# KTH-RPL/cloth-splatting

Measured on AMD Instinct MI355X. Metric: rasterizer fwd+bwd rendered Mpix/s (scene_1, 800x800), higher is better.
Workload: dtype f32

## Files before the change

cloth-splatting_amd/csrc/csplat_image.hip:

```cpp
#include "csplat_common.h"
#include <math.h>
#include <stdlib.h>

namespace {
constexpr int BW = 64, BH = 16, R5 = 5;
struct Taps { float w[11]; };

__global__ __launch_bounds__(256) void k_blur11(int H, int W, Taps taps, const float *__restrict__ in, float *__restrict__ out) {
    __shared__ float s_in[(BH + 2 * R5)][BW + 2 * R5 + 1];
    __shared__ float s_h[(BH + 2 * R5)][BW + 1];
    const size_t img = (size_t)blockIdx.z * H * W;
    const int x0 = blockIdx.x * BW, y0 = blockIdx.y * BH;
    for (int t = threadIdx.x; t < (BH + 2 * R5) * (BW + 2 * R5); t += 256) {
        const int ry = t / (BW + 2 * R5), rx = t - ry * (BW + 2 * R5);
        const int y = y0 + ry - R5, x = x0 + rx - R5;
        s_in[ry][rx] = (y >= 0 && y < H && x >= 0 && x < W) ? in[img + (size_t)y * W + x] : 0.f;
    }
    __syncthreads();
    for (int t = threadIdx.x; t < (BH + 2 * R5) * BW; t += 256) {
        const int ry = t / BW, rx = t - ry * BW;
        float a = 0.f;
#pragma unroll
        for (int k = 0; k < 11; k++) a += taps.w[k] * s_in[ry][rx + k];
        s_h[ry][rx] = a;
// ... 326 lines not shown
#pragma unroll
        for (int o = 32; o > 0; o >>= 1) t += __shfl_xor(t, o, 64);
        __syncthreads();
        if ((threadIdx.x & 63) == 0) s_red[threadIdx.x >> 6] = t;
        __syncthreads();
        float r = 0.f;
        for (int k = 0; k < SSIM_THREADS / 64; k++) r += s_red[k];
        return r;
    };
    const float ssim_sum = block_sum(partial, 0, nwg);
    const float l1_sum = block_sum(partial + nwg, 0, nwg);
    const int n_batch = planes / channels;
    double psnr_sum = 0.0;
    for (int b = 0; b < n_batch; b++) {
        const float q = block_sum(partial + 2 * nwg, (size_t)b * channels * per_plane, (size_t)(b + 1) * channels * per_plane);
        const float mse = q / ((float)channels * (float)H * (float)W);
        psnr_sum += (double)(20.f * log10f(1.f / sqrtf(mse)));
    }
    if (threadIdx.x == 0) {
        const float n = (float)planes * (float)H * (float)W;
        const float l1 = l1_sum / n;
        const float image_loss = masked ? l1 + lam * (ssim_sum / n) : l1 + lam * (1.f - ssim_sum / n);
        out[0] = img_weight * image_loss + (add ? add_weight * add[0] : 0.f);
        out[1] = psnr_scale * (float)psnr_sum;
        out[2] = image_loss;
        out[3] = l1;
    }
}

constexpr int L1_BLOCKS = 256, L1_THREADS = 1024;
__global__ __launch_bounds__(L1_THREADS) void k_l1(int64_t n, const float *__restrict__ a, const float *__restrict__ b,
                                                    float inv_n, float *__restrict__ partial, float *__restrict__ grad,
                                                    const float *__restrict__ mask, int64_t hw, int channels, int mask_channels,
                                                    signed char *__restrict__ sign8) {
    __shared__ float s_red[L1_THREADS / 64];
    float acc = 0.f;
    auto sg = [&](float d) { return d > 0.f ? inv_n : (d < 0.f ? -inv_n : 0.f); };
    auto s8 = [&](float d) { return (signed char)(d > 0.f ? 1 : (d < 0.f ? -1 : 0)); };
    auto moff = [&](int64_t e) {
        const int64_t plane = e / hw;
        return (mask_channels == 1 ? plane / channels : plane) * hw + (e - plane * hw);
    };
    const bool al = ((((uintptr_t)a | (uintptr_t)b | (uintptr_t)grad | (uintptr_t)mask) & 15u) == 0);
    const int64_t n4 = ((mask && (hw & 3)) || !al) ? 0 : n >> 2;
    auto one = [&](int64_t i, const float4 x, const float4 y) {
        float d0 = x.x - y.x, d1 = x.y - y.y, d2 = x.z - y.z, d3 = x.w - y.w;
        if (mask) {
            const float4 m = *reinterpret_cast<const float4 *>(mask + moff(i << 2));
            d0 *= m.x; d1 *= m.y; d2 *= m.z; d3 *= m.w;
            acc += (fabsf(d0) + fabsf(d1)) + (fabsf(d2) + fabsf(d3));
            if (grad) reinterpret_cast<float4 *>(grad)[i] = make_float4(sg(d0) * m.x, sg(d1) * m.y, sg(d2) * m.z, sg(d3) * m.w);
        } else {
            acc += (fabsf(d0) + fabsf(d1)) + (fabsf(d2) + fabsf(d3));
            if (grad) reinterpret_cast<float4 *>(grad)[i] = make_float4(sg(d0), sg(d1), sg(d2), sg(d3));
        }
        if (sign8) reinterpret_cast<char4 *>(sign8)[i] = make_char4(s8(d0), s8(d1), s8(d2), s8(d3));
    };
    const int64_t stride = (int64_t)gridDim.x * L1_THREADS;
    int64_t i = (int64_t)blockIdx.x * L1_THREADS + threadIdx.x;
    for (; i + 3 * stride < n4; i += 4 * stride) {
        const float4 x0 = reinterpret_cast<const float4 *>(a)[i], y0 = reinterpret_cast<const float4 *>(b)[i];
        const float4 x1 = reinterpret_cast<const float4 *>(a)[i + stride], y1 = reinterpret_cast<const float4 *>(b)[i + stride];
        const float4 x2 = reinterpret_cast<const float4 *>(a)[i + 2 * stride], y2 = reinterpret_cast<const float4 *>(b)[i + 2 * stride];
        const float4 x3 = reinterpret_cast<const float4 *>(a)[i + 3 * stride], y3 = reinterpret_cast<const float4 *>(b)[i + 3 * stride];
        one(i, x0, y0);
        one(i + stride, x1, y1);
        one(i + 2 * stride, x2, y2);
        one(i + 3 * stride, x3, y3);
    }
    for (; i + stride < n4; i += 2 * stride) {
        const float4 x0 = reinterpret_cast<const float4 *>(a)[i], y0 = reinterpret_cast<const float4 *>(b)[i];
        const float4 x1 = reinterpret_cast<const float4 *>(a)[i + stride], y1 = reinterpret_cast<const float4 *>(b)[i + stride];
        one(i, x0, y0);
        one(i + stride, x1, y1);
    }
    if (i < n4) one(i, reinterpret_cast<const float4 *>(a)[i], reinterpret_cast<const float4 *>(b)[i]);
    for (int64_t i = (n4 << 2) + (int64_t)blockIdx.x * L1_THREADS + threadIdx.x; i < n; i += (int64_t)gridDim.x * L1_THREADS) {
        float d = a[i] - b[i];
        float m = 1.f;
        if (mask) { m = mask[moff(i)]; d *= m; }
        acc += fabsf(d);
        if (grad) grad[i] = sg(d) * m;
        if (sign8) sign8[i] = s8(d);
    }
#pragma unroll
    for (int o = 32; o > 0; o >>= 1) acc += __shfl_xor(acc, o, 64);
    if ((threadIdx.x & 63) == 0) s_red[threadIdx.x >> 6] = acc;
    __syncthreads();
    if (threadIdx.x == 0) { float t_ = 0.f; for (int k_ = 0; k_ < L1_THREADS / 64; k_++) t_ += s_red[k_]; partial[blockIdx.x] = t_; }
}
__global__ __launch_bounds__(L1_BLOCKS) void k_l1_finish(int nparts, const float *__restrict__ partial, float inv_n, float *__restrict__ loss) {
    __shared__ float s[L1_BLOCKS];
    s[threadIdx.x] = (int)threadIdx.x < nparts ? partial[threadIdx.x] : 0.f;
    __syncthreads();
    if (threadIdx.x == 0) {
        float tt = 0.f;
        for (int g = 0; g < L1_BLOCKS / 16; g++) {
            float t = 0.f;
            for (int k = 0; k < 16; k++) t += s[16 * g + k];
            tt += t;
        }
        *loss = tt * inv_n;
    }
}
constexpr int GL_THREADS = 256, GL_MAX_BLOCKS = 1024, GL_VIEWS = 16;
struct GeomTable {
    const float *D[GL_VIEWS], *A[GL_VIEWS], *Z[GL_VIEWS], *S[GL_VIEWS], *M[GL_VIEWS];
};
__device__ __forceinline__ unsigned geom_code(float r, float w) {
    if (r != r || w != w) return 3u;
    const int sr = (r > 0.f) - (r < 0.f), sw = (w > 0.f) - (w < 0.f);
    return (unsigned)(sr * sw + 1);
}
__device__ __forceinline__ float geom_sign(unsigned code) { return code == 3u ? __builtin_nanf("") : (float)((int)code - 1); }
__device__ __forceinline__ bool geom_valid(float z) { return z > 0.f && z < __builtin_inff(); }

template <bool HAS_Z, bool HAS_S>
__device__ __forceinline__ unsigned geom_pixel(float d, float a, float z, float s, float m, float &acc_d, float &acc_s) {
    unsigned code_d = 1u, code_s = 1u;
    if (HAS_Z) {
        const float w = geom_valid(z) ? m : 0.f;
        const bool on = w != 0.f;
        const float r = fmaf(-a, z, d);
        acc_d += on ? fabsf(r * w) : 0.f;
        code_d = on ? geom_code(r, w) : 1u;
    }
    if (HAS_S) {
        const bool on = m != 0.f;
        const float r = a - s;
        acc_s += on ? fabsf(r * m) : 0.f;
        code_s = on ? geom_code(r, m) : 1u;
    }
    return code_d | (code_s << 2);
}

// ... 167 lines not shown
__global__ __launch_bounds__(256) void k_l1_bwd(int64_t n, const signed char *__restrict__ sign8, const float *__restrict__ g, float inv_n,
                                                const float *__restrict__ mask, int64_t hw, int channels, int mask_channels,
                                                float *__restrict__ out) {
    const float sc = g[0] * inv_n;
    auto moff = [&](int64_t e) {
        const int64_t plane = e / hw;
        return (mask_channels == 1 ? plane / channels : plane) * hw + (e - plane * hw);
    };
    const int64_t n4 = ((mask && (hw & 3)) || ((uintptr_t)mask & 15u)) ? 0 : n >> 2;
    const int64_t stride = (int64_t)gridDim.x * 256;
    for (int64_t i = (int64_t)blockIdx.x * 256 + threadIdx.x; i < n4; i += stride) {
        const char4 s = reinterpret_cast<const char4 *>(sign8)[i];
        float4 o = make_float4(sc * (float)s.x, sc * (float)s.y, sc * (float)s.z, sc * (float)s.w);
        if (mask) {
            const float4 m = *reinterpret_cast<const float4 *>(mask + moff(i << 2));
            o.x *= m.x; o.y *= m.y; o.z *= m.z; o.w *= m.w;
        }
        reinterpret_cast<float4 *>(out)[i] = o;
    }
    for (int64_t i = (n4 << 2) + (int64_t)blockIdx.x * 256 + threadIdx.x; i < n; i += stride)
        out[i] = sc * (float)sign8[i] * (mask ? mask[moff(i)] : 1.f);
}

static int l1_launch(void *stream, int64_t n, const float *a, const float *b, void *scratch, float *loss, float *grad,
                     const float *mask, int64_t hw, int channels, int mask_channels, const char *who, signed char *sign8 = nullptr) {
    CSPLAT_REQUIRE(n > 0 && a && b && scratch && loss, "csplat_l1: bad arguments");
    CSPLAT_REQUIRE((((uintptr_t)a | (uintptr_t)b | (uintptr_t)grad | (uintptr_t)mask) & 3u) == 0, "csplat_l1: operands must be 4-byte aligned");
    const bool al = ((((uintptr_t)a | (uintptr_t)b | (uintptr_t)grad | (uintptr_t)mask) & 15u) == 0);
    float *partial = (float *)scratch;
    const int64_t units = ((mask && (hw & 3)) || !al) ? n : n / 4;
    const int64_t work = (units + L1_THREADS - 1) / L1_THREADS;
    const int grid = (int)(work < 1 ? 1 : (work > L1_BLOCKS ? L1_BLOCKS : work));
    CSPLAT_REQUIRE(((uintptr_t)sign8 & 3u) == 0, "csplat_l1: the sign buffer must be 4-byte aligned");
    k_l1<<<grid, L1_THREADS, 0, (hipStream_t)stream>>>(n, a, b, 1.0f / (float)n, partial, grad, mask, hw, channels, mask_channels, sign8);
    LAUNCH_CHECK();
    k_l1_finish<<<1, L1_BLOCKS, 0, (hipStream_t)stream>>>(grid, partial, 1.0f / (float)n, loss);
    LAUNCH_CHECK();
    (void)who;
    return 0;
}

extern "C" int csplat_l1(void *stream, int64_t n, const float *a, const float *b, void *scratch, float *loss, float *grad) {
    return l1_launch(stream, n, a, b, scratch, loss, grad, nullptr, 1, 1, 1, "csplat_l1");
}

extern "C" int csplat_l1_masked(void *stream, int64_t n_batch, int channels, int64_t hw, const float *a, const float *b,
                                const float *mask, int mask_channels, void *scratch, float *loss, float *grad) {
    CSPLAT_REQUIRE(n_batch > 0 && channels > 0 && hw > 0 && mask, "csplat_l1_masked: bad arguments");
    CSPLAT_REQUIRE(mask_channels == 1 || mask_channels == channels, "csplat_l1_masked: the mask has 1 plane per image or one per channel");
    return l1_launch(stream, n_batch * channels * hw, a, b, scratch, loss, grad, mask, hw, channels, mask_channels, "csplat_l1_masked");
}

extern "C" int csplat_l1_signs(void *stream, int64_t n_batch, int channels, int64_t hw, const float *a, const float *b, const float *mask,
                               int mask_channels, void *scratch, float *loss, signed char *sign8) {
    CSPLAT_REQUIRE(n_batch > 0 && channels > 0 && hw > 0 && sign8, "csplat_l1_signs: bad arguments");
    CSPLAT_REQUIRE(!mask || mask_channels == 1 || mask_channels == channels, "csplat_l1_signs: the mask has 1 plane per image or one per channel");
    return l1_launch(stream, n_batch * channels * hw, a, b, scratch, loss, nullptr, mask, hw, channels, mask ? mask_channels : 1, "csplat_l1_signs", sign8);
}
extern "C" int csplat_l1_signs_bwd(void *stream, int64_t n_batch, int channels, int64_t hw, const signed char *sign8, const float *mask,
                                   int mask_channels, const float *g_scalar, float *out) {
    CSPLAT_REQUIRE(n_batch > 0 && channels > 0 && hw > 0 && sign8 && g_scalar && out, "csplat_l1_signs_bwd: bad arguments");
    CSPLAT_REQUIRE(((uintptr_t)out & 15u) == 0 && (((uintptr_t)sign8 | (uintptr_t)mask) & 3u) == 0, "csplat_l1_signs_bwd: operands must be aligned");
    const int64_t n = n_batch * channels * hw;
    const int64_t work = (n / 4 + 255) / 256;
    const int grid = (int)(work < 1 ? 1 : (work > 4096 ? 4096 : work));
    k_l1_bwd<<<grid, 256, 0, (hipStream_t)stream>>>(n, sign8, g_scalar, 1.0f / (float)n, mask, hw, channels, mask ? mask_channels : 1, out);
    LAUNCH_CHECK();
    return 0;
}
// ... 209 lines not shown
```

cloth-splatting_amd/csrc/csplat_raster.hip:

```cpp
#include "csplat_common.h"

#include <atomic>
#include <cstring>
#include <chrono>
#include <mutex>
#include <type_traits>

#include "csplat_raster_math.h"
#include "csplat_raster_k1.h"
#include "csplat_raster_binning.h"
#include "csplat_raster_k5b_k6.h"

namespace {

constexpr int ACC_STRIDE = 16;

#define CSPLAT_ROWMASK_OP(OP, dst, src0, src1, RM)                                                                                  \
    asm("s_nop 1\n\tv_" OP "_f32_dpp %0, %1, %2 quad_perm:[0,1,2,3] row_mask:" RM " bank_mask:0xf" : "+v"(dst) : "v"(src0), "v"(src1))
__device__ __forceinline__ void rows_scan_mul(float f, float Tin, float &Tr, float &Tout) {
    const auto s16 = __builtin_amdgcn_permlane16_swap(__float_as_uint(f), __float_as_uint(f), false, false);
    const float ev = __uint_as_float(s16[0]), od = __uint_as_float(s16[1]);
    const float pr = ev * od;
    const auto s32 = __builtin_amdgcn_permlane32_swap(__float_as_uint(pr), __float_as_uint(pr), false, false);
    const float lo = __uint_as_float(s32[0]), hi = __uint_as_float(s32[1]);
// ... 730 lines not shown
        std::lock_guard<std::mutex> lk(g_ticket_mu);
        for (int i = 0; i < MAX_TICKETS && tk < 0; i++)
            if (!g_tickets[i].used) tk = i;
        if (tk >= 0) g_tickets[tk].used = true;
    }
    CSPLAT_REQUIRE(tk >= 0, "csplat_forward_begin: more than 64 forwards begun and not finished");
    FwdTicket &t = g_tickets[tk];
    t.s = s; t.P = P; t.W = W; t.H = H; t.tiles = tiles; t.nb = cdiv(P > 0 ? P : 1, BUCKET_G); t.can_bucket = can_bucket;
    t.use_mail = false; t.tag = 0; t.mb_host = nullptr; t.mb_dev = nullptr;
    if (can_bucket && !dbg(CSPLAT_DEBUG_NO_MAILBOX) && mail_init()) {
        t.use_mail = true;
        t.tag = g_mail.next.fetch_add(1);
        if (t.tag == 0) t.tag = g_mail.next.fetch_add(1);
        const int slot = (int)(t.tag % MAIL_SLOTS);
        t.mb_host = g_mail.host + slot * MAIL_WORDS;
        t.mb_dev = g_mail.dev + slot * MAIL_WORDS;
    }
    t.cam = cam; t.g = geom_view(gbase, P); t.gbase = gbase; t.ibase = ibase;
    t.ranges = im.ranges; t.n_contrib = im.n_contrib; t.final_T = im.final_T; t.info = im.info;
    t.table = table; t.bg = bg; t.radii = radii; t.alloc = alloc; t.alloc_ctx = alloc_ctx;
    t.D = D; t.M = M; t.means3D = means3D; t.shs = shs; t.colors_precomp = colors_precomp; t.opacities = opacities; t.scales = scales;
    t.scale_modifier = scale_modifier; t.rotations = rotations; t.cov3D_precomp = cov3D_precomp;
    t.aa = (prefiltered & CSPLAT_ANTIALIAS) != 0;
    *ticket_out = tk;
    return 0;
}

static int nocull_mode() { return dbg(CSPLAT_DEBUG_NO_CULLING) ? 1 : dbg(CSPLAT_DEBUG_CULL_RADIUS_X4) ? 2 : 0; }

static int begin_launch(const FwdTicket &t) {
    hipStream_t s = t.s;
    const int P = t.P, tiles = t.tiles, nb = t.nb;
    if (!t.can_bucket) HIP_TRY(hipMemsetAsync(t.ranges, 0, (size_t)tiles * 8, s));
    if (P > 0) {
        ProfScope ps(PROF_K1, s);
        const bool stage = t.shs != nullptr && t.M == 16 && ((uintptr_t)t.shs & 15u) == 0;
        if (t.aa && stage)
            k_preprocess_aa<true><<<cdiv(P, 256), 256, 0, s>>>(P, t.D, t.M, t.means3D, t.shs, t.colors_precomp, t.opacities, t.scales,
                                                                t.scale_modifier, t.rotations, t.cov3D_precomp, t.cam, t.g, t.radii, nocull_mode());
        else if (t.aa)
            k_preprocess_aa<false><<<cdiv(P, 256), 256, 0, s>>>(P, t.D, t.M, t.means3D, t.shs, t.colors_precomp, t.opacities, t.scales,
                                                                 t.scale_modifier, t.rotations, t.cov3D_precomp, t.cam, t.g, t.radii, nocull_mode());
        else if (stage)
            k_preprocess<true><<<cdiv(P, 256), 256, 0, s>>>(P, t.D, t.M, t.means3D, t.shs, t.colors_precomp, t.opacities, t.scales,
                                                             t.scale_modifier, t.rotations, t.cov3D_precomp, t.cam, t.g, t.radii, nocull_mode());
        else
            k_preprocess<false><<<cdiv(P, 256), 256, 0, s>>>(P, t.D, t.M, t.means3D, t.shs, t.colors_precomp, t.opacities, t.scales,
                                                              t.scale_modifier, t.rotations, t.cov3D_precomp, t.cam, t.g, t.radii, nocull_mode());
        LAUNCH_CHECK();
    }
    if (t.can_bucket) {
        ProfScope ps(PROF_K2, s);
        if (P > 0) {
            k_tile_count<<<nb, BUCKET_G, (size_t)tiles * 4, s>>>(P, tiles, t.g.xy, t.radii, t.cam, t.table);
            LAUNCH_CHECK();
        } else {
            HIP_TRY(hipMemsetAsync(t.table, 0, (size_t)nb * tiles * 4, s));
        }
        uint32_t *tile_cnt = t.table + (size_t)nb * tiles;
        k_tile_colscan<<<cdiv(tiles, 256), 256, 0, s>>>(tiles, nb, t.table, tile_cnt);
        LAUNCH_CHECK();
        k_tile_scan<<<1, 1024, 0, s>>>(tiles, tile_cnt, t.ranges, t.info, t.mb_dev, t.tag);
        LAUNCH_CHECK();
    }
    return 0;
}

static bool begin_views_compatible(int V, const int *tk) {
    if (V < 1 || V > RASTER_MAX_VIEWS || dbg(CSPLAT_DEBUG_PER_VIEW_LAUNCHES)) return false;
    const FwdTicket &a = g_tickets[tk[0]];
    if (a.P <= 0 || !a.can_bucket || !a.shs || a.colors_precomp || a.cov3D_precomp || !a.scales || !a.rotations) return false;
    for (int i = 1; i < V; i++) {
        const FwdTicket &w = g_tickets[tk[i]];
        if (w.P != a.P || w.D != a.D || w.M != a.M || w.W != a.W || w.H != a.H || w.shs != a.shs || w.opacities != a.opacities ||
            w.scales != a.scales || w.scale_modifier != a.scale_modifier || w.colors_precomp || w.cov3D_precomp || !w.rotations ||
            !w.can_bucket || w.aa != a.aa)
            return false;
    }
    return true;
}
static int begin_launch_views(int V, const int *tk, hipStream_t join) {
    const FwdTicket &a = g_tickets[tk[0]];
    const int P = a.P, tiles = a.tiles, nb = a.nb;
    K1Table tab;
    tab.n = V;
    for (int i = 0; i < V; i++) {
        const FwdTicket &t = g_tickets[tk[i]];
        K1View &k = tab.v[i];
        k.means3D = t.means3D; k.rotations = t.rotations; k.cam = t.cam; k.g = t.g; k.radii = t.radii; k.table = t.table;
        k.info = t.info; k.mailbox = t.mb_dev; k.ranges = t.ranges; k.tag = t.tag;
    }
    {
        ProfScope ps(PROF_K1, join);
        const bool stage = a.M == 16 && ((uintptr_t)a.shs & 15u) == 0;
        if (a.aa && stage)
            k_preprocess_views_aa<true><<<cdiv(P, K1V_G), 256, 0, join>>>(P, a.D, a.M, a.shs, a.opacities, a.scales, a.scale_modifier, tab,
                                                                        nocull_mode());
        else if (a.aa)
            k_preprocess_views_aa<false><<<cdiv(P, K1V_G), 256, 0, join>>>(P, a.D, a.M, a.shs, a.opacities, a.scales, a.scale_modifier, tab,
                                                                         nocull_mode());
        else if (stage)
            k_preprocess_views<true><<<cdiv(P, K1V_G), 256, 0, join>>>(P, a.D, a.M, a.shs, a.opacities, a.scales, a.scale_modifier, tab,
                                                                     nocull_mode());
        else
            k_preprocess_views<false><<<cdiv(P, K1V_G), 256, 0, join>>>(P, a.D, a.M, a.shs, a.opacities, a.scales, a.scale_modifier, tab,
                                                                      nocull_mode());
        LAUNCH_CHECK();
    }
    {
        ProfScope ps(PROF_K2, join);
        k_tile_count_views<<<dim3(nb, V), BUCKET_G, (size_t)tiles * 4, join>>>(P, tiles, tab);
        LAUNCH_CHECK();
        k_tile_colscan_views<<<dim3(cdiv(tiles, 256), V), 256, 0, join>>>(tiles, nb, tab);
        LAUNCH_CHECK();
        k_tile_scan_views<<<V, 1024, 0, join>>>(tiles, nb, tab);
        LAUNCH_CHECK();
    }
    return 0;
}

int csplat_forward_begin(void *stream, int P, int D, int M, const float *bg, int W, int H, const float *means3D,
                         const float *shs, const float *colors_precomp, const float *opacities, const float *scales,
                         float scale_modifier, const float *rotations, const float *cov3D_precomp, const float *view,
                         const float *proj, const float *campos, float tanfovx, float tanfovy, int prefiltered,
                         csplat_alloc_fn alloc, void *alloc_ctx, int32_t *radii, int *ticket_out) {
    CSPLAT_REQUIRE(!(prefiltered & CSPLAT_ANTIALIAS), "csplat_forward / csplat_forward_begin: CSPLAT_ANTIALIAS needs a csplat_view entry point "
                                                      "(csplat_forward_views*), whose backward knows the bit");
    if (int rc = begin_prepare(stream, P, D, M, bg, W, H, means3D, shs, colors_precomp, opacities, scales, scale_modifier, rotations,
                               cov3D_precomp, view, proj, campos, tanfovx, tanfovy, prefiltered, alloc, alloc_ctx, radii, ticket_out))
        return rc;
    const int rc = begin_launch(g_tickets[*ticket_out]);
    if (rc) {
        std::lock_guard<std::mutex> lk(g_ticket_mu);
        g_tickets[*ticket_out].used = false;
    }
    return rc;
}

static int finish_read(const FwdTicket &t, uint32_t host_info[3], hipStream_t launched_on = nullptr) {
    hipStream_t s = launched_on ? launched_on : t.s;
    host_info[0] = host_info[1] = host_info[2] = 0;
    if (t.can_bucket) {
        bool got = false;
        if (t.use_mail) {
            const auto t0 = std::chrono::steady_clock::now();
            unsigned spins = 0;
            while (!(got = (t.mb_host[2] == t.tag))) {
                if ((++spins & 0x3FFu) == 0 &&
// ... 1134 lines not shown
```

cloth-splatting_amd/csrc/csplat_raster_binning.h:

```cpp
#pragma once

namespace {

__global__ __launch_bounds__(256) void k_emit_keys(int P, const float2 *__restrict__ xy, const float *__restrict__ depth,
                                                    const uint32_t *__restrict__ offsets,
                                                    const int32_t *__restrict__ radii, Cam cam,
                                                    uint64_t *__restrict__ keys, uint32_t *__restrict__ ids) {
    const int i = blockIdx.x * blockDim.x + threadIdx.x;
    if (i >= P) return;
    const int rad = radii[i];
    if (rad <= 0) return;
    uint32_t off = (i == 0) ? 0u : offsets[i - 1];
    const float2 p = xy[i];
    int minx, miny, maxx, maxy;
    tile_rect(p.x, p.y, rad, cam, minx, miny, maxx, maxy);
    const uint32_t dbits = __float_as_uint(depth[i]);
    for (int y = miny; y < maxy; y++)
        for (int x = minx; x < maxx; x++) {
            keys[off] = ((uint64_t)(uint32_t)(y * cam.gx + x) << 32) | dbits;
            ids[off] = (uint32_t)i;
            off++;
        }
}

__global__ __launch_bounds__(256) void k_tile_ranges(int64_t R, const uint64_t *__restrict__ keys, int2 *__restrict__ ranges) {
    const int64_t i = (int64_t)blockIdx.x * blockDim.x + threadIdx.x;
    if (i >= R) return;
    const uint32_t t = (uint32_t)(keys[i] >> 32);
    if (i == 0) ranges[t].x = 0;
    else {
        const uint32_t tp = (uint32_t)(keys[i - 1] >> 32);
        if (tp != t) { ranges[tp].y = (int)i; ranges[t].x = (int)i; }
    }
    if (i == R - 1) ranges[t].y = (int)R;
}

constexpr int BUCKET_CAP = 8192;
constexpr int BUCKET_TILES = 12288;
constexpr int BUCKET_G = 1024;

__device__ __forceinline__ void tile_count_body(int P, int tiles, const float2 *__restrict__ xy,
                                                const int32_t *__restrict__ radii, const Cam &cam,
                                                uint32_t *__restrict__ table) {
    extern __shared__ uint32_t s_hist[];
    for (int t = threadIdx.x; t < tiles; t += BUCKET_G) s_hist[t] = 0u;
    __syncthreads();
    const int i = blockIdx.x * BUCKET_G + threadIdx.x;
    if (i < P) {
        const int rad = radii[i];
        if (rad > 0) {
            const float2 p = xy[i];
            int minx, miny, maxx, maxy;
            tile_rect(p.x, p.y, rad, cam, minx, miny, maxx, maxy);
            for (int y = miny; y < maxy; y++)
                for (int x = minx; x < maxx; x++) atomicAdd(&s_hist[y * cam.gx + x], 1u);
        }
    }
    __syncthreads();
    uint32_t *row = table + (size_t)blockIdx.x * tiles;
    for (int t = threadIdx.x; t < tiles; t += BUCKET_G) row[t] = s_hist[t];
}
__global__ __launch_bounds__(BUCKET_G) void k_tile_count(int P, int tiles, const float2 *__restrict__ xy,
                                                          const int32_t *__restrict__ radii, Cam cam,
                                                          uint32_t *__restrict__ table) {
    tile_count_body(P, tiles, xy, radii, cam, table);
}
__global__ __launch_bounds__(BUCKET_G) void k_tile_count_views(int P, int tiles, K1Table tab) {
    const K1View &w = tab.v[blockIdx.y];
    tile_count_body(P, tiles, w.g.xy, w.radii, w.cam, w.table);
}

__device__ __forceinline__ void tile_colscan_body(int tiles, int nb, uint32_t *__restrict__ table, uint32_t *__restrict__ cnt) {
    const int t = blockIdx.x * 256 + threadIdx.x;
    if (t >= tiles) return;
    uint32_t run = 0;
    int b = 0;
    for (; b + 8 <= nb; b += 8) {
        uint32_t v[8];
#pragma unroll
        for (int u = 0; u < 8; u++) v[u] = table[(size_t)(b + u) * tiles + t];
#pragma unroll
        for (int u = 0; u < 8; u++) { table[(size_t)(b + u) * tiles + t] = run; run += v[u]; }
    }
    for (; b < nb; b++) { const uint32_t v = table[(size_t)b * tiles + t]; table[(size_t)b * tiles + t] = run; run += v; }
    cnt[t] = run;
}
__global__ __launch_bounds__(256) void k_tile_colscan(int tiles, int nb, uint32_t *__restrict__ table, uint32_t *__restrict__ cnt) {
    tile_colscan_body(tiles, nb, table, cnt);
}
__global__ __launch_bounds__(256) void k_tile_colscan_views(int tiles, int nb, K1Table tab) {
    uint32_t *table = tab.v[blockIdx.y].table;
    tile_colscan_body(tiles, nb, table, table + (size_t)nb * tiles);
}

constexpr int INFO_BUSY = 64;
constexpr int LPT_BINS = 512;
constexpr int TSCAN_ITEMS = BUCKET_TILES / 1024;
__device__ __forceinline__ void tile_scan_body(int tiles, const uint32_t *__restrict__ cnt, int2 *__restrict__ ranges,
                                               uint32_t *__restrict__ info, volatile uint32_t *mailbox, uint32_t tag) {
    __shared__ unsigned long long s_w[17];
    __shared__ uint32_t s_max[16];
    __shared__ uint32_t s_bin[LPT_BINS + 1];
    const int lane = threadIdx.x & 63, w = threadIdx.x >> 6;
    uint32_t *busy = info + INFO_BUSY;
    uint32_t *lpt = busy + tiles + 4;
    const int per = (tiles + 1023) / 1024, t0 = threadIdx.x * per;
    uint32_t c[TSCAN_ITEMS];
#pragma unroll
    for (int k = 0; k < TSCAN_ITEMS; k++) c[k] = (k < per && t0 + k < tiles) ? cnt[t0 + k] : 0u;
    for (int i = threadIdx.x; i <= LPT_BINS; i += 1024) s_bin[i] = 0u;
    uint32_t mx = 0;
    unsigned long long v0 = 0ull;
#pragma unroll
    for (int k = 0; k < TSCAN_ITEMS; k++) { mx = max(mx, c[k]); v0 += (unsigned long long)c[k] | ((unsigned long long)(c[k] ? 1u : 0u) << 32); }
    unsigned long long inc = v0;
#pragma unroll
    for (int d = 1; d < 64; d <<= 1) { const unsigned long long o = __shfl_up(inc, d, 64); if (lane >= d) inc += o; }
    if (lane == 63) s_w[w] = inc;
    __syncthreads();
    if (w == 0) {
        unsigned long long v = lane < 16 ? s_w[lane] : 0ull, vi = v;
#pragma unroll
        for (int d = 1; d < 16; d <<= 1) { const unsigned long long o = __shfl_up(vi, d, 64); if (lane >= d) vi += o; }
        if (lane < 16) s_w[lane] = vi - v;
        if (lane == 15) s_w[16] = vi;
    }
    __syncthreads();
    const unsigned long long carry = s_w[16];
    {
        unsigned long long exl = s_w[w] + inc - v0;
#pragma unroll
        for (int k = 0; k < TSCAN_ITEMS; k++) {
            const int t = t0 + k;
            if (k < per && t < tiles) {
                const uint32_t ex = (uint32_t)exl, nz = (uint32_t)(exl >> 32);
                ranges[t] = c[k] ? make_int2((int)ex, (int)(ex + c[k])) : make_int2(0, 0);
                if (c[k]) {
                    busy[1 + nz] = (uint32_t)t;
                    atomicAdd(&s_bin[LPT_BINS - 1 - min(c[k] >> 4, (uint32_t)(LPT_BINS - 1))], 1u);
                } else {
                    lpt[tiles - 1 - (t - (int)nz)] = (uint32_t)t;
                }
// ... 9 lines not shown
            for (int k = 0; k < LPT_BINS / 64; k++) { v[k] = s_bin[lane * (LPT_BINS / 64) + k]; run += v[k]; }
            uint32_t binc = run;
#pragma unroll
            for (int d = 1; d < 64; d <<= 1) { const uint32_t o = (uint32_t)__shfl_up((int)binc, d, 64); if (lane >= d) binc += o; }
            uint32_t base = binc - run;
#pragma unroll
            for (int k = 0; k < LPT_BINS / 64; k++) { s_bin[lane * (LPT_BINS / 64) + k] = base; base += v[k]; }
        }
        __syncthreads();
#pragma unroll
        for (int k = 0; k < TSCAN_ITEMS; k++)
            if (c[k]) lpt[atomicAdd(&s_bin[LPT_BINS - 1 - min(c[k] >> 4, (uint32_t)(LPT_BINS - 1))], 1u)] = (uint32_t)(t0 + k);
    }
#pragma unroll
    for (int d = 32; d > 0; d >>= 1) mx = max(mx, (uint32_t)__shfl_xor((int)mx, d, 64));
    if (lane == 0) s_max[w] = mx;
    __syncthreads();
    if (threadIdx.x == 0) {
        uint32_t m = 0;
        for (int k = 0; k < 16; k++) m = max(m, s_max[k]);
        info[0] = (uint32_t)carry;
        info[1] = m;
        info[2] = (uint32_t)(carry >> 32);
        busy[0] = (uint32_t)(carry >> 32);
        if (mailbox) {
            mailbox[0] = (uint32_t)carry;
            mailbox[1] = m;
            mailbox[3] = (uint32_t)(carry >> 32);
            __threadfence_system();
            mailbox[2] = tag;
        }
    }
}
__global__ __launch_bounds__(1024) void k_tile_scan(int tiles, const uint32_t *__restrict__ cnt, int2 *__restrict__ ranges,
                                                     uint32_t *__restrict__ info, volatile uint32_t *mailbox, uint32_t tag) {
    tile_scan_body(tiles, cnt, ranges, info, mailbox, tag);
}
__global__ __launch_bounds__(1024) void k_tile_scan_views(int tiles, int nb, K1Table tab) {
    const K1View &w = tab.v[blockIdx.x];
    tile_scan_body(tiles, w.table + (size_t)nb * tiles, w.ranges, w.info, w.mailbox, w.tag);
}

__device__ __forceinline__ void emit_bucket_body(int P, int tiles, const float2 *__restrict__ xy,
                                                 const float *__restrict__ depth, const int32_t *__restrict__ radii,
                                                 const Cam &cam, const uint32_t *__restrict__ table,
                                                 const int2 *__restrict__ ranges, uint64_t *__restrict__ comp) {
    extern __shared__ uint32_t s_base[];
    const uint32_t *row = table + (size_t)blockIdx.x * tiles;
    for (int t = threadIdx.x; t < tiles; t += BUCKET_G) s_base[t] = (uint32_t)ranges[t].x + row[t];
    __syncthreads();
    const int i = blockIdx.x * BUCKET_G + threadIdx.x;
    if (i >= P) return;
    const int rad = radii[i];
    if (rad <= 0) return;
    const float2 p = xy[i];
    int minx, miny, maxx, maxy;
    tile_rect(p.x, p.y, rad, cam, minx, miny, maxx, maxy);
    const uint64_t v = ((uint64_t)__float_as_uint(depth[i]) << 32) | (uint32_t)i;
    for (int y = miny; y < maxy; y++)
        for (int x = minx; x < maxx; x++) comp[atomicAdd(&s_base[y * cam.gx + x], 1u)] = v;
}
__global__ __launch_bounds__(BUCKET_G) void k_emit_bucket(int P, int tiles, const float2 *__restrict__ xy,
                                                           const float *__restrict__ depth, const int32_t *__restrict__ radii,
                                                           Cam cam, const uint32_t *__restrict__ table,
                                                           const int2 *__restrict__ ranges, uint64_t *__restrict__ comp) {
    emit_bucket_body(P, tiles, xy, depth, radii, cam, table, ranges, comp);
}

struct P2View {
    Geom g;
    Cam cam;
    const int32_t *radii;
    const uint32_t *table;
// ... 393 lines not shown
```

cloth-splatting_amd/csrc/csplat_raster_k1.h:

```cpp
#pragma once

namespace {

template <bool STAGE, bool AA = false>
__device__ __forceinline__ void preprocess_body(int P, int D, int M, const float *__restrict__ means3D,
                                                const float *__restrict__ shs,
                                                const float *__restrict__ colors_precomp,
                                                const float *__restrict__ opacities,
                                                const float *__restrict__ scales, float scale_mod,
                                                const float *__restrict__ rotations,
                                                const float *__restrict__ cov3D_precomp, const Cam &cam, const Geom &g,
                                                int32_t *__restrict__ radii, int nocull, const float *s_shrows, int i, int srow) {
#pragma clang fp contract(off)
    if (i >= P) return;
    float depth = 0.f, px = 0.f, py = 0.f, cut = -1.f;
    float4 co = {0.f, 0.f, 0.f, 0.f};
    float rgb[3] = {0.f, 0.f, 0.f};
    float c6[6] = {0.f, 0.f, 0.f, 0.f, 0.f, 0.f};
    uint32_t clampbits = 0, touched = 0;
    int rad = 0;

    const float p[3] = {means3D[3 * i], means3D[3 * i + 1], means3D[3 * i + 2]};
    float pv[3];
    view_point(p, cam.view, pv);
// ... 71 lines not shown
                if (res < 0.f) clampbits |= (1u << ch);
                rgb[ch] = fmaxf(res, 0.f);
            }
        }
        depth = pv[2];
        rad = r;
        px = ix; py = iy;
        float op = opacities[i];
        if constexpr (AA) op = op * aa_h;
        co = make_float4(c * det_inv, -b * det_inv, a * det_inv, op);
        touched = (uint32_t)((maxy - miny) * (maxx - minx));
        const float cancel = 4e-7f * (a * c + b * b) / det;
        cut = cancel < 0.25f ? 2.f * lam1 * logf(255.f * op) * (1.0001f + 2.f * cancel) + 0.01f : 3.0e38f;
        if (nocull == 1) cut = 3.0e38f;
        if (nocull == 2) cut = cut * 4.f + 4.f;
    } while (0);

    g.depth[i] = depth;
    radii[i] = rad;
    g.xy[i] = make_float2(px, py);
    g.conic_opacity[i] = co;
#pragma unroll
    for (int k = 0; k < 3; k++) g.rgb[3 * i + k] = rgb[k];
#pragma unroll
    for (int k = 0; k < 6; k++) g.cov3D[6 * i + k] = c6[k];
    g.clamped[i] = clampbits;
    g.tiles_touched[i] = touched;
    g.cut2[i] = cut;
    g.pack[3 * (size_t)i] = make_float4(px, py, co.x, co.y);
    g.pack[3 * (size_t)i + 1] = make_float4(co.z, co.w, rgb[0], rgb[1]);
    g.pack[3 * (size_t)i + 2] = make_float4(rgb[2], depth, cut, 0.f);
}

template <bool STAGE>
__global__ __launch_bounds__(256) void k_preprocess(int P, int D, int M, const float *__restrict__ means3D,
                                                     const float *__restrict__ shs,
                                                     const float *__restrict__ colors_precomp,
                                                     const float *__restrict__ opacities,
                                                     const float *__restrict__ scales, float scale_mod,
                                                     const float *__restrict__ rotations,
                                                     const float *__restrict__ cov3D_precomp, Cam cam, Geom g,
                                                     int32_t *__restrict__ radii, int nocull) {
    __shared__ float s_shrows[STAGE ? 256 * SH_ROW : 1];
    if (STAGE) {
        const int base = blockIdx.x * 256;
        stage_sh_rows<256>(shs + (size_t)base * 48, min(256, P - base), s_shrows);
        __syncthreads();
    }
    preprocess_body<STAGE>(P, D, M, means3D, shs, colors_precomp, opacities, scales, scale_mod, rotations, cov3D_precomp, cam, g, radii,
                           nocull, s_shrows, (int)(blockIdx.x * blockDim.x + threadIdx.x), (int)threadIdx.x);
}
template <bool STAGE>
__global__ __launch_bounds__(256) void k_preprocess_aa(int P, int D, int M, const float *__restrict__ means3D,
                                                        const float *__restrict__ shs,
                                                        const float *__restrict__ colors_precomp,
                                                        const float *__restrict__ opacities,
                                                        const float *__restrict__ scales, float scale_mod,
                                                        const float *__restrict__ rotations,
                                                        const float *__restrict__ cov3D_precomp, Cam cam, Geom g,
                                                        int32_t *__restrict__ radii, int nocull) {
    __shared__ float s_shrows[STAGE ? 256 * SH_ROW : 1];
    if (STAGE) {
        const int base = blockIdx.x * 256;
        stage_sh_rows<256>(shs + (size_t)base * 48, min(256, P - base), s_shrows);
        __syncthreads();
    }
    preprocess_body<STAGE, true>(P, D, M, means3D, shs, colors_precomp, opacities, scales, scale_mod, rotations, cov3D_precomp, cam, g,
                                 radii, nocull, s_shrows, (int)(blockIdx.x * blockDim.x + threadIdx.x), (int)threadIdx.x);
}

struct K1View {
    const float *means3D, *rotations;
    Cam cam;
    Geom g;
    int32_t *radii;
    uint32_t *table, *info, *mailbox;
    int2 *ranges;
    uint32_t tag;
};
struct K1Table { int n; K1View v[RASTER_MAX_VIEWS]; };

constexpr int K1V_G = 64;
template <bool STAGE>
__global__ __launch_bounds__(256) void k_preprocess_views(int P, int D, int M, const float *__restrict__ shs,
                                                           const float *__restrict__ opacities,
                                                           const float *__restrict__ scales, float scale_mod, K1Table tab,
                                                           int nocull) {
    __shared__ float s_shrows[STAGE ? K1V_G * SH_ROW : 1];
    const int base = blockIdx.x * K1V_G;
    if (STAGE) {
        stage_sh_rows<256>(shs + (size_t)base * 48, min(K1V_G, P - base), s_shrows);
        __syncthreads();
    }
    const int lane = threadIdx.x & 63;
    for (int vi = threadIdx.x >> 6; vi < tab.n; vi += 4) {
        const K1View &w = tab.v[vi];
        preprocess_body<STAGE>(P, D, M, w.means3D, shs, nullptr, opacities, scales, scale_mod, w.rotations, nullptr, w.cam, w.g, w.radii, nocull,
                               s_shrows, base + lane, lane);
    }
}
template <bool STAGE>
__global__ __launch_bounds__(256) void k_preprocess_views_aa(int P, int D, int M, const float *__restrict__ shs,
                                                              const float *__restrict__ opacities,
                                                              const float *__restrict__ scales, float scale_mod, K1Table tab,
                                                              int nocull) {
    __shared__ float s_shrows[STAGE ? K1V_G * SH_ROW : 1];
    const int base = blockIdx.x * K1V_G;
    if (STAGE) {
        stage_sh_rows<256>(shs + (size_t)base * 48, min(K1V_G, P - base), s_shrows);
        __syncthreads();
    }
    const int lane = threadIdx.x & 63;
    for (int vi = threadIdx.x >> 6; vi < tab.n; vi += 4) {
        const K1View &w = tab.v[vi];
        preprocess_body<STAGE, true>(P, D, M, w.means3D, shs, nullptr, opacities, scales, scale_mod, w.rotations, nullptr, w.cam, w.g, w.radii,
                                     nocull, s_shrows, base + lane, lane);
    }
}

}
```

Before: 4737.

## Fuse tile histogram, column scan and tile scan via atomics and last-block ticket

Replaces the three-kernel binning sequence (per-block tile histogram, column-wise exclusive scan, single-block tile scan) with one kernel. Each block atomically adds its per-tile counts into a global total and keeps the returned base as its offset, and the last block to draw a ticket runs the tile scan. Tile totals and the ticket are zeroed inside the preprocess kernel. The L1 loss finish kernel is likewise folded into the main reduction using a last-block ticket. Both remove kernel launches and the separate colscan pass over memory. In exchange, per-block offsets become nondeterministic, so primitive order within a tile now depends on atomic ordering, and correctness relies on cross-block memory-ordering assumptions.

Result: no change. 4700 (-0.8%).

```diff
diff --git a/cloth-splatting_amd/csrc/csplat_image.hip b/cloth-splatting_amd/csrc/csplat_image.hip
--- a/cloth-splatting_amd/csrc/csplat_image.hip
+++ b/cloth-splatting_amd/csrc/csplat_image.hip
@@ -382,7 +382,7 @@
 __global__ __launch_bounds__(L1_THREADS) void k_l1(int64_t n, const float *__restrict__ a, const float *__restrict__ b,
                                                     float inv_n, float *__restrict__ partial, float *__restrict__ grad,
                                                     const float *__restrict__ mask, int64_t hw, int channels, int mask_channels,
-                                                    signed char *__restrict__ sign8) {
+                                                    signed char *__restrict__ sign8, float *__restrict__ loss) {
     __shared__ float s_red[L1_THREADS / 64];
     float acc = 0.f;
     auto sg = [&](float d) { return d > 0.f ? inv_n : (d < 0.f ? -inv_n : 0.f); };
@@ -437,20 +437,35 @@
     for (int o = 32; o > 0; o >>= 1) acc += __shfl_xor(acc, o, 64);
     if ((threadIdx.x & 63) == 0) s_red[threadIdx.x >> 6] = acc;
     __syncthreads();
-    if (threadIdx.x == 0) { float t_ = 0.f; for (int k_ = 0; k_ < L1_THREADS / 64; k_++) t_ += s_red[k_]; partial[blockIdx.x] = t_; }
-}
-__global__ __launch_bounds__(L1_BLOCKS) void k_l1_finish(int nparts, const float *__restrict__ partial, float inv_n, float *__restrict__ loss) {
-    __shared__ float s[L1_BLOCKS];
-    s[threadIdx.x] = (int)threadIdx.x < nparts ? partial[threadIdx.x] : 0.f;
-    __syncthreads();
+    uint32_t *ticket = reinterpret_cast<uint32_t *>(partial + L1_BLOCKS);
     if (threadIdx.x == 0) {
-        float tt = 0.f;
-        for (int g = 0; g < L1_BLOCKS / 16; g++) {
-            float t = 0.f;
-            for (int k = 0; k < 16; k++) t += s[16 * g + k];
-            tt += t;
-        }
+        float t_ = 0.f;
+        for (int k_ = 0; k_ < L1_THREADS / 64; k_++) t_ += s_red[k_];
+        __hip_atomic_store(partial + blockIdx.x, t_, __ATOMIC_RELAXED, __HIP_MEMORY_SCOPE_AGENT);
+    }
+    if (threadIdx.x < 64) asm volatile("s_waitcnt vmcnt(0)" ::: "memory");
+    __syncthreads();
+    if (threadIdx.x >= 64) return;
+    uint32_t drawn = 0u;
+    if (threadIdx.x == 0) drawn = __hip_atomic_fetch_add(ticket, 1u, __ATOMIC_RELAXED, __HIP_MEMORY_SCOPE_AGENT);
+    if ((uint32_t)__builtin_amdgcn_readfirstlane((int)drawn) != gridDim.x - 1) return;
+    float t = 0.f;
+    if (threadIdx.x < L1_BLOCKS / 16) {
+        float v[16];
+#pragma unroll
+        for (int k = 0; k < 16; k++) {
+            const unsigned idx = 16u * threadIdx.x + k;
+            v[k] = __hip_atomic_load(partial + idx, __ATOMIC_RELAXED, __HIP_MEMORY_SCOPE_AGENT);
+        }
+#pragma unroll
+        for (int k = 0; k < 16; k++) t += 16u * threadIdx.x + k < gridDim.x ? v[k] : 0.f;
+    }
+    float tt = 0.f;
+#pragma unroll
+    for (int g = 0; g < L1_BLOCKS / 16; g++) tt += __shfl(t, g, 64);
+    if (threadIdx.x == 0) {
         *loss = tt * inv_n;
+        __hip_atomic_store(ticket, 0u, __ATOMIC_RELAXED, __HIP_MEMORY_SCOPE_AGENT);
     }
 }
 constexpr int GL_THREADS = 256, GL_MAX_BLOCKS = 1024, GL_VIEWS = 16;
@@ -684,9 +699,8 @@
     const int64_t work = (units + L1_THREADS - 1) / L1_THREADS;
     const int grid = (int)(work < 1 ? 1 : (work > L1_BLOCKS ? L1_BLOCKS : work));
     CSPLAT_REQUIRE(((uintptr_t)sign8 & 3u) == 0, "csplat_l1: the sign buffer must be 4-byte aligned");
-    k_l1<<<grid, L1_THREADS, 0, (hipStream_t)stream>>>(n, a, b, 1.0f / (float)n, partial, grad, mask, hw, channels, mask_channels, sign8);
-    LAUNCH_CHECK();
-    k_l1_finish<<<1, L1_BLOCKS, 0, (hipStream_t)stream>>>(grid, partial, 1.0f / (float)n, loss);
+    k_l1<<<grid, L1_THREADS, 0, (hipStream_t)stream>>>(n, a, b, 1.0f / (float)n, partial, grad, mask, hw, channels, mask_channels, sign8,
+                                                       loss);
     LAUNCH_CHECK();
     (void)who;
     return 0;
diff --git a/cloth-splatting_amd/csrc/csplat_raster.hip b/cloth-splatting_amd/csrc/csplat_raster.hip
--- a/cloth-splatting_amd/csrc/csplat_raster.hip
+++ b/cloth-splatting_amd/csrc/csplat_raster.hip
@@ -786,35 +786,36 @@
     hipStream_t s = t.s;
     const int P = t.P, tiles = t.tiles, nb = t.nb;
     if (!t.can_bucket) HIP_TRY(hipMemsetAsync(t.ranges, 0, (size_t)tiles * 8, s));
+    uint32_t *total = t.can_bucket ? t.table + (size_t)nb * tiles : nullptr, *ticket = t.info + INFO_TICKET;
     if (P > 0) {
         ProfScope ps(PROF_K1, s);
         const bool stage = t.shs != nullptr && t.M == 16 && ((uintptr_t)t.shs & 15u) == 0;
         if (t.aa && stage)
             k_preprocess_aa<true><<<cdiv(P, 256), 256, 0, s>>>(P, t.D, t.M, t.means3D, t.shs, t.colors_precomp, t.opacities, t.scales,
-                                                                t.scale_modifier, t.rotations, t.cov3D_precomp, t.cam, t.g, t.radii, nocull_mode());
+                                                                t.scale_modifier, t.rotations, t.cov3D_precomp, t.cam, t.g, t.radii, nocull_mode(),
+                                                                total, tiles, ticket);
         else if (t.aa)
             k_preprocess_aa<false><<<cdiv(P, 256), 256, 0, s>>>(P, t.D, t.M, t.means3D, t.shs, t.colors_precomp, t.opacities, t.scales,
-                                                                 t.scale_modifier, t.rotations, t.cov3D_precomp, t.cam, t.g, t.radii, nocull_mode());
+                                                                 t.scale_modifier, t.rotations, t.cov3D_precomp, t.cam, t.g, t.radii, nocull_mode(),
+                                                                 total, tiles, ticket);
         else if (stage)
             k_preprocess<true><<<cdiv(P, 256), 256, 0, s>>>(P, t.D, t.M, t.means3D, t.shs, t.colors_precomp, t.opacities, t.scales,
-                                                             t.scale_modifier, t.rotations, t.cov3D_precomp, t.cam, t.g, t.radii, nocull_mode());
+                                                             t.scale_modifier, t.rotations, t.cov3D_precomp, t.cam, t.g, t.radii, nocull_mode(),
+                                                             total, tiles, ticket);
         else
             k_preprocess<false><<<cdiv(P, 256), 256, 0, s>>>(P, t.D, t.M, t.means3D, t.shs, t.colors_precomp, t.opacities, t.scales,
-                                                              t.scale_modifier, t.rotations, t.cov3D_precomp, t.cam, t.g, t.radii, nocull_mode());
+                                                              t.scale_modifier, t.rotations, t.cov3D_precomp, t.cam, t.g, t.radii, nocull_mode(),
+                                                              total, tiles, ticket);
         LAUNCH_CHECK();
     }
     if (t.can_bucket) {
         ProfScope ps(PROF_K2, s);
-        if (P > 0) {
-            k_tile_count<<<nb, BUCKET_G, (size_t)tiles * 4, s>>>(P, tiles, t.g.xy, t.radii, t.cam, t.table);
-            LAUNCH_CHECK();
-        } else {
-            HIP_TRY(hipMemsetAsync(t.table, 0, (size_t)nb * tiles * 4, s));
-        }
-        uint32_t *tile_cnt = t.table + (size_t)nb * tiles;
-        k_tile_colscan<<<cdiv(tiles, 256), 256, 0, s>>>(tiles, nb, t.table, tile_cnt);
-        LAUNCH_CHECK();
-        k_tile_scan<<<1, 1024, 0, s>>>(tiles, tile_cnt, t.ranges, t.info, t.mb_dev, t.tag);
+        if (P == 0) {
+            HIP_TRY(hipMemsetAsync(total, 0, (size_t)tiles * 4, s));
+            HIP_TRY(hipMemsetAsync(ticket, 0, 4, s));
+        }
+        k_tile_count<<<nb, BUCKET_G, (size_t)tiles * 4, s>>>(P, tiles, nb, t.g.xy, t.radii, t.cam, t.table, t.ranges, t.info, t.mb_dev,
+                                                             t.tag);
         LAUNCH_CHECK();
     }
     return 0;
@@ -849,25 +850,21 @@
         const bool stage = a.M == 16 && ((uintptr_t)a.shs & 15u) == 0;
         if (a.aa && stage)
             k_preprocess_views_aa<true><<<cdiv(P, K1V_G), 256, 0, join>>>(P, a.D, a.M, a.shs, a.opacities, a.scales, a.scale_modifier, tab,
-                                                                        nocull_mode());
+                                                                        nocull_mode(), tiles, nb);
         else if (a.aa)
             k_preprocess_views_aa<false><<<cdiv(P, K1V_G), 256, 0, join>>>(P, a.D, a.M, a.shs, a.opacities, a.scales, a.scale_modifier, tab,
-                                                                         nocull_mode());
+                                                                         nocull_mode(), tiles, nb);
         else if (stage)
             k_preprocess_views<true><<<cdiv(P, K1V_G), 256, 0, join>>>(P, a.D, a.M, a.shs, a.opacities, a.scales, a.scale_modifier, tab,
-                                                                     nocull_mode());
+                                                                     nocull_mode(), tiles, nb);
         else
             k_preprocess_views<false><<<cdiv(P, K1V_G), 256, 0, join>>>(P, a.D, a.M, a.shs, a.opacities, a.scales, a.scale_modifier, tab,
-                                                                      nocull_mode());
+                                                                      nocull_mode(), tiles, nb);
         LAUNCH_CHECK();
     }
     {
         ProfScope ps(PROF_K2, join);
         k_tile_count_views<<<dim3(nb, V), BUCKET_G, (size_t)tiles * 4, join>>>(P, tiles, tab);
-        LAUNCH_CHECK();
-        k_tile_colscan_views<<<dim3(cdiv(tiles, 256), V), 256, 0, join>>>(tiles, nb, tab);
-        LAUNCH_CHECK();
-        k_tile_scan_views<<<V, 1024, 0, join>>>(tiles, nb, tab);
         LAUNCH_CHECK();
     }
     return 0;
diff --git a/cloth-splatting_amd/csrc/csplat_raster_binning.h b/cloth-splatting_amd/csrc/csplat_raster_binning.h
--- a/cloth-splatting_amd/csrc/csplat_raster_binning.h
+++ b/cloth-splatting_amd/csrc/csplat_raster_binning.h
@@ -39,64 +39,10 @@
 constexpr int BUCKET_TILES = 12288;
 constexpr int BUCKET_G = 1024;
 
-__device__ __forceinline__ void tile_count_body(int P, int tiles, const float2 *__restrict__ xy,
-                                                const int32_t *__restrict__ radii, const Cam &cam,
-                                                uint32_t *__restrict__ table) {
-    extern __shared__ uint32_t s_hist[];
-    for (int t = threadIdx.x; t < tiles; t += BUCKET_G) s_hist[t] = 0u;
-    __syncthreads();
-    const int i = blockIdx.x * BUCKET_G + threadIdx.x;
-    if (i < P) {
-        const int rad = radii[i];
-        if (rad > 0) {
-            const float2 p = xy[i];
-            int minx, miny, maxx, maxy;
-            tile_rect(p.x, p.y, rad, cam, minx, miny, maxx, maxy);
-            for (int y = miny; y < maxy; y++)
-                for (int x = minx; x < maxx; x++) atomicAdd(&s_hist[y * cam.gx + x], 1u);
-        }
-    }
-    __syncthreads();
-    uint32_t *row = table + (size_t)blockIdx.x * tiles;
-    for (int t = threadIdx.x; t < tiles; t += BUCKET_G) row[t] = s_hist[t];
-}
-__global__ __launch_bounds__(BUCKET_G) void k_tile_count(int P, int tiles, const float2 *__restrict__ xy,
-                                                          const int32_t *__restrict__ radii, Cam cam,
-                                                          uint32_t *__restrict__ table) {
-    tile_count_body(P, tiles, xy, radii, cam, table);
-}
-__global__ __launch_bounds__(BUCKET_G) void k_tile_count_views(int P, int tiles, K1Table tab) {
-    const K1View &w = tab.v[blockIdx.y];
-    tile_count_body(P, tiles, w.g.xy, w.radii, w.cam, w.table);
-}
-
-__device__ __forceinline__ void tile_colscan_body(int tiles, int nb, uint32_t *__restrict__ table, uint32_t *__restrict__ cnt) {
-    const int t = blockIdx.x * 256 + threadIdx.x;
-    if (t >= tiles) return;
-    uint32_t run = 0;
-    int b = 0;
-    for (; b + 8 <= nb; b += 8) {
-        uint32_t v[8];
-#pragma unroll
-        for (int u = 0; u < 8; u++) v[u] = table[(size_t)(b + u) * tiles + t];
-#pragma unroll
-        for (int u = 0; u < 8; u++) { table[(size_t)(b + u) * tiles + t] = run; run += v[u]; }
-    }
-    for (; b < nb; b++) { const uint32_t v = table[(size_t)b * tiles + t]; table[(size_t)b * tiles + t] = run; run += v; }
-    cnt[t] = run;
-}
-__global__ __launch_bounds__(256) void k_tile_colscan(int tiles, int nb, uint32_t *__restrict__ table, uint32_t *__restrict__ cnt) {
-    tile_colscan_body(tiles, nb, table, cnt);
-}
-__global__ __launch_bounds__(256) void k_tile_colscan_views(int tiles, int nb, K1Table tab) {
-    uint32_t *table = tab.v[blockIdx.y].table;
-    tile_colscan_body(tiles, nb, table, table + (size_t)nb * tiles);
-}
-
 constexpr int INFO_BUSY = 64;
 constexpr int LPT_BINS = 512;
 constexpr int TSCAN_ITEMS = BUCKET_TILES / 1024;
-__device__ __forceinline__ void tile_scan_body(int tiles, const uint32_t *__restrict__ cnt, int2 *__restrict__ ranges,
+__device__ __forceinline__ void tile_scan_body(int tiles, uint32_t *__restrict__ cnt, int2 *__restrict__ ranges,
                                                uint32_t *__restrict__ info, volatile uint32_t *mailbox, uint32_t tag) {
     __shared__ unsigned long long s_w[17];
     __shared__ uint32_t s_max[16];
@@ -107,7 +53,7 @@
     const int per = (tiles + 1023) / 1024, t0 = threadIdx.x * per;
     uint32_t c[TSCAN_ITEMS];
 #pragma unroll
-    for (int k = 0; k < TSCAN_ITEMS; k++) c[k] = (k < per && t0 + k < tiles) ? cnt[t0 + k] : 0u;
+    for (int k = 0; k < TSCAN_ITEMS; k++) c[k] = (k < per && t0 + k < tiles) ? atomicExch(&cnt[t0 + k], 0u) : 0u;
     for (int i = threadIdx.x; i <= LPT_BINS; i += 1024) s_bin[i] = 0u;
     uint32_t mx = 0;
     unsigned long long v0 = 0ull;
@@ -183,13 +129,54 @@
         }
     }
 }
-__global__ __launch_bounds__(1024) void k_tile_scan(int tiles, const uint32_t *__restrict__ cnt, int2 *__restrict__ ranges,
-                                                     uint32_t *__restrict__ info, volatile uint32_t *mailbox, uint32_t tag) {
-    tile_scan_body(tiles, cnt, ranges, info, mailbox, tag);
-}
-__global__ __launch_bounds__(1024) void k_tile_scan_views(int tiles, int nb, K1Table tab) {
-    const K1View &w = tab.v[blockIdx.x];
-    tile_scan_body(tiles, w.table + (size_t)nb * tiles, w.ranges, w.info, w.mailbox, w.tag);
+constexpr int INFO_TICKET = K1_INFO_TICKET;
+constexpr int TCOUNT_BATCH = 4;
+__device__ __forceinline__ void tile_count_body(int P, int tiles, int nb, const float2 *__restrict__ xy,
+                                                const int32_t *__restrict__ radii, const Cam &cam,
+                                                uint32_t *__restrict__ table, int2 *__restrict__ ranges,
+                                                uint32_t *__restrict__ info, volatile uint32_t *mailbox, uint32_t tag) {
+    extern __shared__ uint32_t s_hist[];
+    __shared__ uint32_t s_last;
+    for (int t = threadIdx.x; t < tiles; t += BUCKET_G) s_hist[t] = 0u;
+    __syncthreads();
+    const int i = blockIdx.x * BUCKET_G + threadIdx.x;
+    if (i < P) {
+        const int rad = radii[i];
+        if (rad > 0) {
+            const float2 p = xy[i];
+            int minx, miny, maxx, maxy;
+            tile_rect(p.x, p.y, rad, cam, minx, miny, maxx, maxy);
+            for (int y = miny; y < maxy; y++)
+                for (int x = minx; x < maxx; x++) atomicAdd(&s_hist[y * cam.gx + x], 1u);
+        }
+    }
+    __syncthreads();
+    uint32_t *row = table + (size_t)blockIdx.x * tiles;
+    uint32_t *total = table + (size_t)nb * tiles;
+    for (int t0 = threadIdx.x; t0 < tiles; t0 += TCOUNT_BATCH * BUCKET_G) {
+        uint32_t c[TCOUNT_BATCH], base[TCOUNT_BATCH] = {};
+#pragma unroll
+        for (int k = 0; k < TCOUNT_BATCH; k++) { const int t = t0 + k * BUCKET_G; c[k] = t < tiles ? s_hist[t] : 0u; }
+#pragma unroll
+        for (int k = 0; k < TCOUNT_BATCH; k++) if (c[k]) base[k] = atomicAdd(&total[t0 + k * BUCKET_G], c[k]);
+#pragma unroll
+        for (int k = 0; k < TCOUNT_BATCH; k++) if (c[k]) row[t0 + k * BUCKET_G] = base[k];
+    }
+    __syncthreads();
+    if (threadIdx.x == 0) s_last = atomicAdd(&info[INFO_TICKET], 1u) == (uint32_t)(nb - 1) ? 1u : 0u;
+    __syncthreads();
+    if (!s_last) return;
+    tile_scan_body(tiles, total, ranges, info, mailbox, tag);
+}
+__global__ __launch_bounds__(BUCKET_G) void k_tile_count(int P, int tiles, int nb, const float2 *__restrict__ xy,
+                                                          const int32_t *__restrict__ radii, Cam cam,
+                                                          uint32_t *__restrict__ table, int2 *__restrict__ ranges,
+                                                          uint32_t *__restrict__ info, volatile uint32_t *mailbox, uint32_t tag) {
+    tile_count_body(P, tiles, nb, xy, radii, cam, table, ranges, info, mailbox, tag);
+}
+__global__ __launch_bounds__(BUCKET_G) void k_tile_count_views(int P, int tiles, K1Table tab) {
+    const K1View &w = tab.v[blockIdx.y];
+    tile_count_body(P, tiles, (int)gridDim.x, w.g.xy, w.radii, w.cam, w.table, w.ranges, w.info, w.mailbox, w.tag);
 }
 
 __device__ __forceinline__ void emit_bucket_body(int P, int tiles, const float2 *__restrict__ xy,
diff --git a/cloth-splatting_amd/csrc/csplat_raster_k1.h b/cloth-splatting_amd/csrc/csplat_raster_k1.h
--- a/cloth-splatting_amd/csrc/csplat_raster_k1.h
+++ b/cloth-splatting_amd/csrc/csplat_raster_k1.h
@@ -127,6 +127,12 @@
     g.pack[3 * (size_t)i + 2] = make_float4(rgb[2], depth, cut, 0.f);
 }
 
+__device__ __forceinline__ void zero_tile_totals(uint32_t *__restrict__ total, int tiles, uint32_t *__restrict__ ticket) {
+    if (!total) return;
+    for (int t = blockIdx.x * 256 + threadIdx.x; t < tiles; t += gridDim.x * 256) total[t] = 0u;
+    if (blockIdx.x == 0 && threadIdx.x == 0) *ticket = 0u;
+}
+
 template <bool STAGE>
 __global__ __launch_bounds__(256) void k_preprocess(int P, int D, int M, const float *__restrict__ means3D,
                                                      const float *__restrict__ shs,
@@ -135,8 +141,10 @@
                                                      const float *__restrict__ scales, float scale_mod,
                                                      const float *__restrict__ rotations,
                                                      const float *__restrict__ cov3D_precomp, Cam cam, Geom g,
-                                                     int32_t *__restrict__ radii, int nocull) {
+                                                     int32_t *__restrict__ radii, int nocull, uint32_t *__restrict__ total, int tiles,
+                                                     uint32_t *__restrict__ ticket) {
     __shared__ float s_shrows[STAGE ? 256 * SH_ROW : 1];
+    zero_tile_totals(total, tiles, ticket);
     if (STAGE) {
         const int base = blockIdx.x * 256;
         stage_sh_rows<256>(shs + (size_t)base * 48, min(256, P - base), s_shrows);
@@ -153,8 +161,10 @@
                                                         const float *__restrict__ scales, float scale_mod,
                                                         const float *__restrict__ rotations,
                                                         const float *__restrict__ cov3D_precomp, Cam cam, Geom g,
-                                                        int32_t *__restrict__ radii, int nocull) {
+                                                        int32_t *__restrict__ radii, int nocull, uint32_t *__restrict__ total, int tiles,
+                                                        uint32_t *__restrict__ ticket) {
     __shared__ float s_shrows[STAGE ? 256 * SH_ROW : 1];
+    zero_tile_totals(total, tiles, ticket);
     if (STAGE) {
         const int base = blockIdx.x * 256;
         stage_sh_rows<256>(shs + (size_t)base * 48, min(256, P - base), s_shrows);
@@ -164,6 +174,7 @@
                                  radii, nocull, s_shrows, (int)(blockIdx.x * blockDim.x + threadIdx.x), (int)threadIdx.x);
 }
 
+constexpr int K1_INFO_TICKET = 3;
 struct K1View {
     const float *means3D, *rotations;
     Cam cam;
@@ -180,9 +191,11 @@
 __global__ __launch_bounds__(256) void k_preprocess_views(int P, int D, int M, const float *__restrict__ shs,
                                                            const float *__restrict__ opacities,
                                                            const float *__restrict__ scales, float scale_mod, K1Table tab,
-                                                           int nocull) {
+                                                           int nocull, int tiles, int nb) {
     __shared__ float s_shrows[STAGE ? K1V_G * SH_ROW : 1];
     const int base = blockIdx.x * K1V_G;
+    if ((int)blockIdx.x * 256 < tiles)
+        for (int vi = 0; vi < tab.n; vi++) zero_tile_totals(tab.v[vi].table + (size_t)nb * tiles, tiles, tab.v[vi].info + K1_INFO_TICKET);
     if (STAGE) {
         stage_sh_rows<256>(shs + (size_t)base * 48, min(K1V_G, P - base), s_shrows);
         __syncthreads();
@@ -198,9 +211,11 @@
 __global__ __launch_bounds__(256) void k_preprocess_views_aa(int P, int D, int M, const float *__restrict__ shs,
                                                               const float *__restrict__ opacities,
                                                               const float *__restrict__ scales, float scale_mod, K1Table tab,
-                                                              int nocull) {
+                                                              int nocull, int tiles, int nb) {
     __shared__ float s_shrows[STAGE ? K1V_G * SH_ROW : 1];
     const int base = blockIdx.x * K1V_G;
+    if ((int)blockIdx.x * 256 < tiles)
+        for (int vi = 0; vi < tab.n; vi++) zero_tile_totals(tab.v[vi].table + (size_t)nb * tiles, tiles, tab.v[vi].info + K1_INFO_TICKET);
     if (STAGE) {
         stage_sh_rows<256>(shs + (size_t)base * 48, min(K1V_G, P - base), s_shrows);
         __syncthreads();
```
